# nktoan/h-edit

Hardware: AMD Instinct MI355X
Metric: edited images/sec (512^2, 50 steps, K Langevin) (higher is better)
Workload: dtype bf16

## Files before the change

h-edit_amd/csrc/c_api.hip:

```cpp
#include "../../include/hedit.h"
#include <exception>
#include <map>
#include <mutex>
#include <new>
#include <set>
#include <utility>

#include "common.h"
#include "kernels.h"

static thread_local std::string g_last_error;
void hedit_set_error(const std::string& msg) { g_last_error = msg; }

int hedit_abi_catch() noexcept {
  try {
    try {
      throw;
    } catch (const std::bad_alloc&) {
      g_last_error = "out of host memory inside libhedit_hip";
    } catch (const std::exception& e) {
      g_last_error = std::string("C++ exception inside libhedit_hip: ") + e.what();
    } catch (...) {
      g_last_error = "unknown C++ exception inside libhedit_hip";
    }
// ... 335 lines not shown
                       int B, int N, int heads, int d, const hedit_p2p_plan* plan, float* store, void* stream) try {
  ARG_CHECK(q && k && vt && out && plan, "cross_attn args");
  CrossAttnParams p{};
  p.q = reinterpret_cast<const bf16_t*>(q); p.ldq = ldq;
  p.k = reinterpret_cast<const bf16_t*>(k); p.ldk = ldk;
  p.vt = reinterpret_cast<const bf16_t*>(vt); p.ldvt = (long)ldvt;
  p.out = reinterpret_cast<bf16_t*>(out); p.ldo = ldo;
  p.B = B; p.N = N; p.heads = heads; p.d = d;
  p.n_pairs = plan->n_pairs; p.pair_src = plan->pair_src; p.pair_tar = plan->pair_tar;
  p.mixT = reinterpret_cast<const bf16_t*>(plan->mixT); p.bvec = plan->bvec;
  p.singles = plan->singles; p.n_single = plan->n_single;
  p.store = store;
  return cross_attn_launch(p, S(stream));
} catch (...) { return hedit_abi_catch(); }

int hedit_k_attn_probs(const void* q, int ldq, const void* k, int ldk, float* probs, int B, int N, int M, int kstride,
                       int heads, int d, void* stream) try {
  ARG_CHECK(q && k && probs, "attn_probs args");
  AttnProbsParams p{};
  p.q = reinterpret_cast<const bf16_t*>(q); p.ldq = ldq;
  p.k = reinterpret_cast<const bf16_t*>(k); p.ldk = ldk;
  p.probs = probs; p.B = B; p.N = N; p.M = M; p.kstride = kstride; p.heads = heads; p.d = d;
  return attn_probs_launch(p, S(stream));
} catch (...) { return hedit_abi_catch(); }

int hedit_k_attn_apply(const float* probs, const void* vt, int64_t ldvt, void* out, int ldo, int B, int N, int M,
                       int kstride, int heads, int d, void* stream) try {
  ARG_CHECK(probs && vt && out, "attn_apply args");
  AttnProbsParams p{};
  p.probs = const_cast<float*>(probs);
  p.vt = reinterpret_cast<const bf16_t*>(vt); p.ldvt = (long)ldvt;
  p.out = reinterpret_cast<bf16_t*>(out); p.ldo = ldo;
  p.B = B; p.N = N; p.M = M; p.kstride = kstride; p.heads = heads; p.d = d;
  return attn_apply_launch(p, S(stream));
} catch (...) { return hedit_abi_catch(); }

int hedit_k_pack_conv3x3(const float* w, void* out, int O, int I, void* stream) try {
  ARG_CHECK(w && out, "pack args");
  return pack_conv3x3_launch(w, reinterpret_cast<bf16_t*>(out), O, I, S(stream));
} catch (...) { return hedit_abi_catch(); }

int hedit_k_f32_to_bf16(const float* x, void* y, int64_t n, void* stream) try {
  ARG_CHECK(x && y, "cast args");
  return f32_to_bf16_launch(x, reinterpret_cast<bf16_t*>(y), (long)n, S(stream));
} catch (...) { return hedit_abi_catch(); }

int hedit_k_groupnorm_stats(const void* x, void* y, const float* gamma, const float* beta, int B, int HW, int C, int G,
                            float eps, int silu, void* ws, float* stats, void* stream) try {
  ARG_CHECK(x && y && gamma && beta && ws && stats, "groupnorm_stats args");
  return groupnorm_launch(reinterpret_cast<const bf16_t*>(x), reinterpret_cast<bf16_t*>(y), gamma, beta, B, HW, C, G,
                          eps, silu, reinterpret_cast<float*>(ws), S(stream), stats);
} catch (...) { return hedit_abi_catch(); }

size_t hedit_k_groupnorm_bwd_ws_bytes(int B, int HW, int C) { return groupnorm_bwd_ws_bytes(B, HW, C); }

int hedit_k_groupnorm_bwd(const void* x, const void* dy, const void* add, void* dx, const float* gamma, const float* beta,
                          const float* stats, int B, int HW, int C, int G, int silu, void* ws, void* stream) try {
  ARG_CHECK(x && dy && dx && gamma && beta && stats && ws, "groupnorm_bwd args");
  return groupnorm_bwd_launch(reinterpret_cast<const bf16_t*>(x), reinterpret_cast<const bf16_t*>(dy),
                              reinterpret_cast<const bf16_t*>(add), reinterpret_cast<bf16_t*>(dx), gamma, beta, stats, B, HW, C,
                              G, silu, reinterpret_cast<float*>(ws), S(stream));
} catch (...) { return hedit_abi_catch(); }

int hedit_k_softmax_rows(const float* s, void* p, int64_t rows, int N, float scale, void* stream) try {
  ARG_CHECK(s && p, "softmax_rows args");
  return softmax_rows_launch(s, reinterpret_cast<bf16_t*>(p), (long)rows, N, scale, S(stream));
} catch (...) { return hedit_abi_catch(); }

int hedit_k_softmax_blockdiag(const float* s, void* p, int64_t rows, int T, int ld, float scale, void* stream) try {
  ARG_CHECK(s && p, "softmax_blockdiag args");
  return softmax_blockdiag_launch(s, reinterpret_cast<bf16_t*>(p), (long)rows, T, ld, scale, S(stream));
} catch (...) { return hedit_abi_catch(); }

int hedit_k_softmax_bwd(const void* p, const float* dp, void* ds, int64_t rows, int N, float scale, void* stream) try {
  ARG_CHECK(p && dp && ds, "softmax_bwd args");
  return softmax_bwd_launch(reinterpret_cast<const bf16_t*>(p), dp, reinterpret_cast<bf16_t*>(ds), (long)rows, N, scale, S(stream));
} catch (...) { return hedit_abi_catch(); }

int hedit_k_transpose(const void* src, void* dst, int R, int C, void* stream) try {
  ARG_CHECK(src && dst, "transpose args");
  return transpose_bf16_launch(reinterpret_cast<const bf16_t*>(src), reinterpret_cast<bf16_t*>(dst), R, C, S(stream));
} catch (...) { return hedit_abi_catch(); }

int hedit_k_sum2x2(const void* du, void* dx, int B, int H, int W, int C, void* stream) try {
  ARG_CHECK(du && dx, "sum2x2 args");
  return sum2x2_launch(reinterpret_cast<const bf16_t*>(du), reinterpret_cast<bf16_t*>(dx), B, H, W, C, S(stream));
} catch (...) { return hedit_abi_catch(); }

int hedit_k_pack_conv3x3_dgrad(const float* w, void* out, int O, int I, void* stream) try {
  ARG_CHECK(w && out, "pack args");
  return pack_conv3x3_dgrad_launch(w, reinterpret_cast<bf16_t*>(out), O, I, S(stream));
} catch (...) { return hedit_abi_catch(); }

int hedit_k_pack_conv3x3_s2_dgrad(const float* w, void* out, int O, int I, void* stream) try {
  ARG_CHECK(w && out, "pack args");
  return pack_conv3x3_s2_dgrad_launch(w, reinterpret_cast<bf16_t*>(out), O, I, S(stream));
} catch (...) { return hedit_abi_catch(); }

int hedit_k_conv3x3_s2_dgrad(const void* dy, const void* w_packed, void* dx, int B, int Hin, int Win, int O, int I, void* stream) try {
  ARG_CHECK(dy && w_packed && dx, "conv3x3_s2_dgrad args");
  return conv3x3_s2_dgrad_launch(reinterpret_cast<const bf16_t*>(dy), reinterpret_cast<const bf16_t*>(w_packed),
                                 reinterpret_cast<bf16_t*>(dx), B, Hin, Win, O, I, S(stream));
} catch (...) { return hedit_abi_catch(); }

int hedit_k_slice_add(const void* src, int ld, int off, int c, void* dst, int64_t rows, int accumulate, void* stream) try {
  ARG_CHECK(src && dst && rows >= 0, "slice_add args");
// ... 78 lines not shown
```

h-edit_amd/csrc/kernels.h:

```cpp
#pragma once
#include "common.h"

struct GemmParams {
  const bf16_t* A;
  const bf16_t* W;
  int M, N, K;
  int lda;
  int mode;
  int Hin, Win, Cin, Hout, Wout;
  const float* bias;
  const bf16_t* residual;
  int ldr;
  bf16_t* C;
  int ldc;
  float* partial;
  int splits, kt_per_split;
  int n_fastest;
  const bf16_t* zeros;
  unsigned a_bytes, w_bytes;
  int geglu;
  int asym;
  float* raw_f32;
  int chunk_kt;
  const float *ln_gamma, *ln_beta;
// ... 11 lines not shown
int gemm_pick_splits(int M, int N, int K, int force);
int gemm_canonical_chunk(int M_nom, int N_nom, int K);
int gemm_plan_splits(int M, int N, int K, int chunk_kt);
size_t gemm_partial_bytes(int M, int N, int splits);
int gemm_launch(GemmParams p, int splits, float* partial_ws, hipStream_t st);
bool pgemm_supported(const GemmParams& p, int splits, int bn);
int pgemm_launch(const GemmParams& p, int bn, hipStream_t st);
bool pconv_supported(const GemmParams& p, int splits, int bn);
int pconv_launch(const GemmParams& p, int bn, hipStream_t st);

struct FfnParams {
  const bf16_t* x; long ldx;
  const float* gamma; const float* beta; float eps;
  const bf16_t* stream;
  const float* bias1p;
  const float* bias2;
  bf16_t* out; long ldo;
  int M, C;
  const bf16_t* a; long lda;
  const bf16_t* r2; long ldr2;
  const float* bias_pre; const float* bias_post;
};
struct LinChainParams {
  const bf16_t* a; long lda;
  const bf16_t* r1; long ldr1;
  const float* bias_pre;
  const float* gamma; const float* beta; float eps;
  const bf16_t* stream;
  bf16_t* out_mid; long ldmid;
  bf16_t* out; long ldo;
  int M, C;
  const float* gn_ss; int rows_per_image;
  bf16_t* out_q; long ldq; bf16_t* out_k; long ldk;
};
int lin_chain_launch(const LinChainParams& c, hipStream_t st);
int lin_chain_launch_sched(const LinChainParams& c, int sched, hipStream_t st);
size_t lin_chain_stream_bytes(int layers);
int lin_chain_pack_launch(const float* w, int layer, float scale, int layers, bf16_t* stream, hipStream_t st);
int ffn_fused_channels();
size_t ffn_stream_bytes(int pre, int post);
size_t ffn_bias_bytes();
int ffn_pack_launch(const float* w, int which, int pre, int post, bf16_t* stream, hipStream_t st);
int ffn_pack_bias_launch(const float* b1, float* out, hipStream_t st);
int ffn_fused_launch(const FfnParams& f, hipStream_t st);

#define HEDIT_MAXW 77
#define HEDIT_WPAD 96
#define HEDIT_CTXP 80

size_t groupnorm_ws_bytes(int B, int HW, int C);
int groupnorm_launch(const bf16_t* x, bf16_t* y, const float* gamma, const float* beta, int B,
                     int HW, int C, int G, float eps, int silu, float* ws, hipStream_t st,
                     float* stats = nullptr);
bool groupnorm_from_parts_supported(int HW, int C, int G);
size_t groupnorm_from_parts_ws_bytes(int B);
int groupnorm_from_parts_launch(const bf16_t* x, bf16_t* y, const float* gamma, const float* beta, int B, int HW, int C, int G,
                                float eps, int silu, const float* part_a, int ca, const float* part_b, int cb, float* ws,
                                hipStream_t st);
int groupnorm_affine_launch(const bf16_t* x, const float* gamma, const float* beta, int B, int HW, int C, int G, float eps,
                            float* ws, hipStream_t st, const float** ss_out);
int layernorm_launch(const bf16_t* x, bf16_t* y, const float* gamma, const float* beta, long rows,
                     int C, float eps, hipStream_t st);
bool splitk_reduce_ln_supported(int C);
int splitk_reduce_ln_launch(const float* partial, int splits, const float* bias, const bf16_t* residual, int ldr, bf16_t* out,
                            bf16_t* y, const float* gamma, const float* beta, long rows, int C, float eps, hipStream_t st);
int geglu_launch(const bf16_t* x, bf16_t* y, long rows, int inner, hipStream_t st);
#define HEDIT_ROWMAP_MAX 512
struct RowMap { uint16_t src[HEDIT_ROWMAP_MAX]; };
int concat_launch(const bf16_t* a, int ca, const bf16_t* b, int cb, bf16_t* y, long rows, hipStream_t st,
                  const RowMap* b_map = nullptr, int rows_per_image = 0);
int gather_rows_launch(const void* const* src, void* const* dst, int n, int B, long row_bytes, const RowMap& map, hipStream_t st);
int f32_to_bf16_launch(const float* x, bf16_t* y, long n, hipStream_t st);
int ctx_pad_launch(const float* x, bf16_t* y, int B, int dim, hipStream_t st);
int gemv_launch(const bf16_t* W, const float* x, const float* b0, const float* b1, float* out,
                int N, int K, int silu, hipStream_t st);
int copy_rows_launch(bf16_t* x, const int* src, int B, long row_elems, hipStream_t st);
int timestep_embed_launch(float t, float* out, int dim, hipStream_t st);
int timestep_embed_ddpm_launch(float t, float* out, int dim, hipStream_t st);
int conv_in_launch(const float* x, const float* w, const float* bias, bf16_t* y, int B, int Cin,
                   int H, int W, int Cout, hipStream_t st);
int conv_out_launch(const bf16_t* x, const bf16_t* w, const float* bias, float* y, int B, int H,
                    int W, int C, int Cout, hipStream_t st);
int rows_to_nchw_launch(const float* src, const float* bias, float* dst, int B, long HW, int ld, int Cout, hipStream_t st);
int softmax_rows_launch(const float* s, bf16_t* p, long rows, int N, float scale, hipStream_t st);
int softmax_blockdiag_launch(const float* s, bf16_t* p, long rows, int T, int ld, float scale, hipStream_t st);
int mix1x1_nchw_launch(const float* x, const float* w, const float* bias, float* y, int B, int Cin, int Cout, long HW,
                       float pre_scale, hipStream_t st);
int quant_mean_launch(const bf16_t* h, const float* w, const float* bias, float* y, int B, long HW, int Cm, int Cout, hipStream_t st);
int pack_linear_launch(const float* w, bf16_t* out, long n, float scale, hipStream_t st);
int pack_conv3x3_launch(const float* w_oihw, bf16_t* out, int O, int I, hipStream_t st);
int pack_geglu_rows_launch(const float* w, bf16_t* out_bf16, float* out_f32, int rows, int K, hipStream_t st);

size_t groupnorm_bwd_ws_bytes(int B, int HW, int C);
int groupnorm_bwd_launch(const bf16_t* x, const bf16_t* dy, const bf16_t* add, bf16_t* dx, const float* gamma,
                         const float* beta, const float* stats, int B, int HW, int C, int G, int silu, float* ws,
                         hipStream_t st, bool any_width = false);
int softmax_bwd_launch(const bf16_t* p, const float* dp, bf16_t* ds, long rows, int N, float scale, hipStream_t st);
int transpose_bf16_launch(const bf16_t* src, bf16_t* dst, int R, int C, hipStream_t st);
int sum2x2_launch(const bf16_t* du, bf16_t* dx, int B, int H, int W, int C, hipStream_t st);
int pack_conv3x3_dgrad_launch(const float* w_oihw, bf16_t* out, int O, int I, hipStream_t st);
int pack_linear_t_launch(const float* w, bf16_t* out, int O, int I, hipStream_t st, float scale = 1.f);
int flip_oihw_launch(const float* w, float* out, int O, int I, int k, hipStream_t st);
int layernorm_bwd_launch(const bf16_t* x, const bf16_t* dy, const bf16_t* add, bf16_t* dx, const float* gamma, long rows, int C,
                         float eps, hipStream_t st);
int geglu_bwd_launch(const bf16_t* x, const bf16_t* dy, bf16_t* dx, long rows, int inner, hipStream_t st);

// ... 135 lines not shown
```

h-edit_amd/csrc/norm.hip:

```cpp
#include <stdlib.h>
#include "common.h"
#include "kernels.h"

namespace {


constexpr int GN_MAXV = 2;

__global__ __launch_bounds__(256) void gn_partial_kernel(const bf16_t* __restrict__ x, float* __restrict__ part,
                                                         int HW, int C, int G, int nslab) {
  extern __shared__ float lds[];
  const int CV = C / 8;
  const int slab = blockIdx.x, b = blockIdx.y;
  const int pix_per = (HW + nslab - 1) / nslab;
  const int p0 = slab * pix_per;
  int p1 = p0 + pix_per;
  if (p1 > HW) p1 = HW;
  const int R = CV <= 256 ? 256 / CV : 1;
  const int r = CV <= 256 ? threadIdx.x / CV : 0;
  const int cv0 = CV <= 256 ? threadIdx.x % CV : threadIdx.x;
  const bool active = r < R;
  float s[GN_MAXV][8], q[GN_MAXV][8];
#pragma unroll
  for (int v = 0; v < GN_MAXV; ++v)
// ... 550 lines not shown
#pragma unroll
      for (int j = 0; j < 8; ++j) acc[co] += f[j] * ww[j];
    }
  }
  for (int co = 0; co < Cout; ++co) {
    float v = wave_sum(acc[co]);
    if (lane == 0) y[(((long)b * Cout + co) * H + oy) * Wd + ox] = v + bias[co];
  }
}

__global__ __launch_bounds__(256) void gn_small_kernel(const bf16_t* __restrict__ x, bf16_t* __restrict__ y,
                                                       const float* __restrict__ gamma, const float* __restrict__ beta,
                                                       int HW, int C, int G, float eps, int silu, float* __restrict__ stats) {
  extern __shared__ uint32_t gs_pairs[];
  __shared__ float red[8];
  const int g = blockIdx.x, b = blockIdx.y, tid = threadIdx.x;
  const int cpg = C / G, ppp = cpg / 2;
  const int npair = HW * ppp;
  const uint32_t* xin = reinterpret_cast<const uint32_t*>(x + (long)b * HW * C + g * cpg);
  float s = 0.f, q = 0.f;
  for (int i = tid; i < npair; i += 256) {
    const int pix = i / ppp, j = i - pix * ppp;
    const uint32_t u = xin[(long)pix * (C / 2) + j];
    gs_pairs[i] = u;
    const float a = st_lo(u), c = st_hi(u);
    s += a; s += c;
    q += a * a; q += c * c;
  }
  s = wave_sum(s);
  q = wave_sum(q);
  if ((tid & 63) == 0) { red[(tid >> 6) * 2] = s; red[(tid >> 6) * 2 + 1] = q; }
  __syncthreads();
  s = ((red[0] + red[2]) + red[4]) + red[6];
  q = ((red[1] + red[3]) + red[5]) + red[7];
  const float n = (float)HW * (float)cpg;
  const float m = s / n;
  float var = q / n - m * m;
  var = var < 0.f ? 0.f : var;
  const float rstd = rsqrtf(var + eps);
  if (stats && tid == 0) *reinterpret_cast<float2*>(stats + ((long)b * G + g) * 2) = make_float2(m, rstd);
  uint32_t* yout = reinterpret_cast<uint32_t*>(y + (long)b * HW * C + g * cpg);
  for (int i = tid; i < npair; i += 256) {
    const int pix = i / ppp, j = i - pix * ppp;
    const uint32_t u = gs_pairs[i];
    const int c0 = g * cpg + 2 * j;
    const float sc0 = rstd * gamma[c0], sc1 = rstd * gamma[c0 + 1];
    float a = st_lo(u) * sc0 + (beta[c0] - m * sc0);
    float c = st_hi(u) * sc1 + (beta[c0 + 1] - m * sc1);
    if (silu) { a = silu_f(a); c = silu_f(c); }
    yout[(long)pix * (C / 2) + j] = pack_bf16x2(a, c);
  }
}

__global__ __launch_bounds__(256) void gn_fold_kernel(const float* __restrict__ pa, int npa, const float* __restrict__ pb, int npb,
                                                      float* __restrict__ out, int units, int ppg) {
  __shared__ float red[8];
  const int g = blockIdx.x, b = blockIdx.y, tid = threadIdx.x;
  const int total = units * ppg;
  float s = 0.f, q = 0.f;
  for (int e = tid; e < total; e += 256) {
    const int u = e / ppg, j = e - u * ppg;
    const int pr = g * ppg + j;
    const long row = (long)b * units + u;
    const float2 v = pr < npa ? *reinterpret_cast<const float2*>(pa + (row * npa + pr) * 2)
                              : *reinterpret_cast<const float2*>(pb + (row * npb + (pr - npa)) * 2);
    s += v.x;
    q += v.y;
  }
  s = wave_sum(s);
  q = wave_sum(q);
  if ((tid & 63) == 0) { red[(tid >> 6) * 2] = s; red[(tid >> 6) * 2 + 1] = q; }
  __syncthreads();
  if (tid == 0) {
    s = ((red[0] + red[2]) + red[4]) + red[6];
    q = ((red[1] + red[3]) + red[5]) + red[7];
    *reinterpret_cast<float2*>(out + ((long)b * gridDim.x + g) * 2) = make_float2(s, q);
  }
}

int gn_nslab(int B, int HW, int C) {
  (void)B;
  const int CV = C / 8;
  const int R = CV <= 256 ? 256 / CV : 1;
  int n = HW / (R * 8);
  int cap = HW / 256;
  cap = cap < 32 ? 32 : (cap > 64 ? 64 : cap);
  if (HW >= 512 * 512) cap = 128;
  if (n > cap) n = cap;
  if (n < 1) n = 1;
  return n;
}

}

size_t groupnorm_ws_bytes(int B, int HW, int C) {
  const int nslab = gn_nslab(B, HW, C);
  return ((size_t)B * nslab * 64 * 2 + (size_t)B * C * 2) * sizeof(float);
}

int groupnorm_launch(const bf16_t* x, bf16_t* y, const float* gamma, const float* beta, int B, int HW,
                     int C, int G, float eps, int silu, float* ws, hipStream_t st, float* stats) {
  ARG_CHECK(C % 8 == 0 && C % G == 0 && G <= 64, "groupnorm: C % 8, C % G, G <= 64");
  ARG_CHECK(C / 8 <= 256 * GN_MAXV, "groupnorm: C too large");
  if (HW < 1024 && (C / G) % 2 == 0 && (size_t)HW * (C / G) * 2 <= 60 * 1024) {
    hipLaunchKernelGGL(gn_small_kernel, dim3(G, B), dim3(256), (size_t)HW * (C / G) * 2, st, x, y, gamma, beta, HW, C, G, eps, silu, stats);
    LAUNCH_CHECK();
    return HEDIT_OK;
  }
  const int nslab = gn_nslab(B, HW, C);
  float* part = ws;
  float* ss = ws + (size_t)B * nslab * 64 * 2;
  const int CV = C / 8;
  const int R = CV <= 256 ? 256 / CV : 1;
  const size_t lds = (size_t)R * C * 2 * sizeof(float);
  ARG_CHECK(lds <= 64 * 1024, "groupnorm: LDS");
  hipLaunchKernelGGL(gn_partial_kernel, dim3(nslab, B), dim3(256), lds, st, x, part, HW, C, G, nslab);
  LAUNCH_CHECK();
  const long total_v = (long)B * HW * CV;
  const bool rows_form = CV <= 256 && HW >= 1024;
  if (!rows_form || stats) {
    hipLaunchKernelGGL(gn_finalize_kernel, dim3(B), dim3(256), 0, st, part, gamma, beta, ss, HW, C, G, nslab, eps, stats);
    LAUNCH_CHECK();
  }
  if (rows_form) {
    int ns = (int)(4096 / (B > 0 ? B : 1)) + 1;
    const int max_ns = HW / (R * 8) > 0 ? HW / (R * 8) : 1;
    if (ns > max_ns) ns = max_ns;
    {
      int pix = HW / ns / (4 * R) * (4 * R);
      if (pix < 4 * R) pix = 4 * R;
      ns = (HW + pix - 1) / pix;
    }
    hipLaunchKernelGGL(gn_apply_rows_kernel, dim3(ns, B), dim3(256), 0, st, x, y, part, gamma, beta, HW, C, G, nslab, eps, silu, ns);
    LAUNCH_CHECK();
    return HEDIT_OK;
  }
  hipLaunchKernelGGL(gn_apply_kernel, dim3(ew_grid(total_v)), dim3(256), 0, st, x, y, ss, total_v, HW, C, silu);
  LAUNCH_CHECK();
  return HEDIT_OK;
}

bool groupnorm_from_parts_supported(int HW, int C, int G) {
  return HW >= 1024 && HW % 128 == 0 && C % 8 == 0 && C / 8 <= 256 && C % G == 0 && (C / G) % 2 == 0 && G <= 64;
}
size_t groupnorm_from_parts_ws_bytes(int B) { return (size_t)B * 64 * 2 * sizeof(float); }

int groupnorm_from_parts_launch(const bf16_t* x, bf16_t* y, const float* gamma, const float* beta, int B, int HW, int C, int G,
                                float eps, int silu, const float* part_a, int ca, const float* part_b, int cb, float* ws,
                                hipStream_t st) {
  ARG_CHECK(groupnorm_from_parts_supported(HW, C, G), "groupnorm_from_parts: shape");
  ARG_CHECK(part_a && ca > 0 && ca % 2 == 0 && cb >= 0 && cb % 2 == 0 && ca + cb == C && (cb == 0) == (part_b == nullptr),
            "groupnorm_from_parts: the pair statistics must cover the C channels");
  hipLaunchKernelGGL(gn_fold_kernel, dim3(G, B), dim3(256), 0, st, part_a, ca / 2, part_b, cb / 2, ws, HW / 128, C / G / 2);
  LAUNCH_CHECK();
  const int CV = C / 8, R = 256 / CV;
  int ns = (int)(4096 / (B > 0 ? B : 1)) + 1;
  const int max_ns = HW / (R * 8) > 0 ? HW / (R * 8) : 1;
// ... 342 lines not shown
```

h-edit_amd/hedit/_lib.py:

```python
import ctypes as C
import os

_HERE = os.path.dirname(os.path.abspath(__file__))
STORAGE = os.environ.get("HEDIT_STORAGE", "bf16").lower()
if STORAGE not in ("bf16", "f16"):
    raise ValueError(f"HEDIT_STORAGE must be bf16 or f16, not {STORAGE!r}")
LIB_PATH = os.path.join(_HERE, "libhedit_hip_f16.so" if STORAGE == "f16" else "libhedit_hip.so")
HEDIT_MAX_LEVELS = 8


class UnetCfg(C.Structure):
    _fields_ = [("in_channels", C.c_int), ("out_channels", C.c_int), ("sample_size", C.c_int),
                ("n_levels", C.c_int),
                ("block_out_channels", C.c_int * HEDIT_MAX_LEVELS),
                ("down_has_attn", C.c_int * HEDIT_MAX_LEVELS),
                ("up_has_attn", C.c_int * HEDIT_MAX_LEVELS),
                ("layers_per_block", C.c_int), ("cross_attention_dim", C.c_int),
                ("heads", C.c_int), ("norm_num_groups", C.c_int)]


class VaeCfg(C.Structure):
    _fields_ = [("in_channels", C.c_int), ("latent_channels", C.c_int), ("n_levels", C.c_int),
                ("block_out_channels", C.c_int * 4), ("layers_per_block", C.c_int),
                ("norm_num_groups", C.c_int)]
# ... 226 lines not shown
                                 C.c_void_p]),
    "hedit_k_gemm_ws_bytes": (C.c_size_t, [C.c_int, C.c_int, C.c_int, C.c_int]),
    "hedit_k_gemm_canonical_chunk": (C.c_int, [C.c_int, C.c_int, C.c_int]),
    "hedit_k_gemm_plan_splits": (C.c_int, [C.c_int, C.c_int, C.c_int, C.c_int]),
    "hedit_k_gemm": (C.c_int, [C.c_void_p, C.c_void_p, C.c_void_p, C.c_void_p, C.c_void_p] + [C.c_int] * 13 +
                     [C.c_void_p, C.c_void_p]),
    "hedit_k_conv_gn": (C.c_int, [C.c_void_p, C.c_void_p, C.c_void_p, C.c_void_p, C.c_void_p] + [C.c_int] * 12 +
                        [C.c_void_p, C.c_void_p, C.c_void_p]),
    "hedit_k_groupnorm_from_parts": (C.c_int, [C.c_void_p, C.c_void_p, C.c_void_p, C.c_void_p, C.c_int, C.c_int, C.c_int, C.c_int,
                                               C.c_float, C.c_int, C.c_void_p, C.c_int, C.c_void_p, C.c_int, C.c_void_p, C.c_void_p]),
    "hedit_k_pack_geglu": (C.c_int, [C.c_void_p, C.c_void_p, C.c_void_p, C.c_void_p, C.c_int, C.c_int, C.c_void_p]),
    "hedit_k_gemm_geglu": (C.c_int, [C.c_void_p, C.c_void_p, C.c_void_p, C.c_void_p, C.c_int, C.c_int, C.c_int,
                                     C.c_int, C.c_int, C.c_void_p]),
    "hedit_test_set_flags": (C.c_int, [C.c_int]),
    "hedit_storage_is_f16": (C.c_int, []),
    "hedit_k_lin_chain_stream_bytes": (C.c_size_t, [C.c_int]),
    "hedit_k_lin_chain_pack": (C.c_int, [C.c_void_p, C.c_void_p, C.c_void_p, C.c_void_p, C.c_float, C.c_void_p, C.c_void_p]),
    "hedit_k_lin_chain": (C.c_int, [C.c_void_p, C.c_int64, C.c_void_p, C.c_int64, C.c_void_p, C.c_int, C.c_void_p, C.c_void_p, C.c_void_p,
                                    C.c_float, C.c_void_p, C.c_void_p, C.c_int64, C.c_void_p, C.c_int64, C.c_void_p, C.c_int64,
                                    C.c_void_p, C.c_int64, C.c_int, C.c_int, C.c_void_p]),
    "hedit_k_lin_chain_sched": (C.c_int, [C.c_void_p, C.c_int64, C.c_void_p, C.c_int64, C.c_void_p, C.c_int, C.c_void_p, C.c_void_p, C.c_void_p,
                                          C.c_float, C.c_void_p, C.c_void_p, C.c_int64, C.c_void_p, C.c_int64, C.c_void_p, C.c_int64,
                                          C.c_void_p, C.c_int64, C.c_int, C.c_int, C.c_int, C.c_void_p]),
    "hedit_k_groupnorm_affine": (C.c_int, [C.c_void_p, C.c_void_p, C.c_void_p, C.c_int, C.c_int, C.c_int, C.c_int, C.c_float, C.c_void_p,
                                           C.c_void_p, C.c_void_p]),
    "hedit_k_ffn_channels": (C.c_int, []),
    "hedit_k_ffn_stream_bytes": (C.c_size_t, [C.c_int]),
    "hedit_k_ffn_bias_bytes": (C.c_size_t, []),
    "hedit_k_ffn_pack": (C.c_int, [C.c_void_p, C.c_void_p, C.c_void_p, C.c_void_p, C.c_void_p, C.c_void_p, C.c_void_p, C.c_void_p]),
    "hedit_k_ffn_chain": (C.c_int, [C.c_void_p, C.c_int64, C.c_void_p, C.c_int64, C.c_void_p, C.c_int64, C.c_void_p, C.c_void_p, C.c_void_p,
                                    C.c_float, C.c_void_p, C.c_void_p, C.c_void_p, C.c_void_p, C.c_void_p, C.c_int64, C.c_int, C.c_int,
                                    C.c_void_p]),
    "hedit_k_ffn_fused": (C.c_int, [C.c_void_p, C.c_int64, C.c_void_p, C.c_void_p, C.c_float, C.c_void_p, C.c_void_p,
                                    C.c_void_p, C.c_void_p, C.c_int64, C.c_int, C.c_int, C.c_void_p]),
    "hedit_k_groupnorm_ws_bytes": (C.c_size_t, [C.c_int, C.c_int, C.c_int]),
    "hedit_k_groupnorm": (C.c_int, [C.c_void_p, C.c_void_p, C.c_void_p, C.c_void_p, C.c_int, C.c_int, C.c_int,
                                    C.c_int, C.c_float, C.c_int, C.c_void_p, C.c_void_p]),
    "hedit_k_layernorm": (C.c_int, [C.c_void_p, C.c_void_p, C.c_void_p, C.c_void_p, C.c_int64, C.c_int,
                                    C.c_float, C.c_void_p]),
    "hedit_k_geglu": (C.c_int, [C.c_void_p, C.c_void_p, C.c_int64, C.c_int, C.c_void_p]),
    "hedit_k_self_attn": (C.c_int, [C.c_void_p, C.c_int, C.c_void_p, C.c_int, C.c_void_p, C.c_int64, C.c_void_p,
                                    C.c_int, C.c_int, C.c_int, C.c_int, C.c_int, C.c_void_p, C.c_void_p, C.c_void_p]),
    "hedit_k_cross_attn": (C.c_int, [C.c_void_p, C.c_int, C.c_void_p, C.c_int, C.c_void_p, C.c_int64, C.c_void_p,
                                     C.c_int, C.c_int, C.c_int, C.c_int, C.c_int, C.POINTER(P2PPlan), C.c_void_p,
                                     C.c_void_p]),
    "hedit_k_attn_probs": (C.c_int, [C.c_void_p, C.c_int, C.c_void_p, C.c_int, C.c_void_p, C.c_int, C.c_int, C.c_int, C.c_int,
                                     C.c_int, C.c_int, C.c_void_p]),
    "hedit_k_attn_apply": (C.c_int, [C.c_void_p, C.c_void_p, C.c_int64, C.c_void_p, C.c_int, C.c_int, C.c_int, C.c_int, C.c_int,
                                     C.c_int, C.c_int, C.c_void_p]),
    "hedit_k_pack_conv3x3": (C.c_int, [C.c_void_p, C.c_void_p, C.c_int, C.c_int, C.c_void_p]),
    "hedit_k_f32_to_bf16": (C.c_int, [C.c_void_p, C.c_void_p, C.c_int64, C.c_void_p]),
    "hedit_k_groupnorm_stats": (C.c_int, [C.c_void_p, C.c_void_p, C.c_void_p, C.c_void_p, C.c_int, C.c_int, C.c_int,
                                          C.c_int, C.c_float, C.c_int, C.c_void_p, C.c_void_p, C.c_void_p]),
    "hedit_k_groupnorm_bwd_ws_bytes": (C.c_size_t, [C.c_int, C.c_int, C.c_int]),
    "hedit_k_groupnorm_bwd": (C.c_int, [C.c_void_p] * 7 + [C.c_int] * 5 + [C.c_void_p, C.c_void_p]),
    "hedit_k_softmax_rows": (C.c_int, [C.c_void_p, C.c_void_p, C.c_int64, C.c_int, C.c_float, C.c_void_p]),
    "hedit_k_softmax_blockdiag": (C.c_int, [C.c_void_p, C.c_void_p, C.c_int64, C.c_int, C.c_int, C.c_float, C.c_void_p]),
    "hedit_k_softmax_bwd": (C.c_int, [C.c_void_p, C.c_void_p, C.c_void_p, C.c_int64, C.c_int, C.c_float, C.c_void_p]),
    "hedit_k_transpose": (C.c_int, [C.c_void_p, C.c_void_p, C.c_int, C.c_int, C.c_void_p]),
    "hedit_k_sum2x2": (C.c_int, [C.c_void_p, C.c_void_p, C.c_int, C.c_int, C.c_int, C.c_int, C.c_void_p]),
    "hedit_k_pack_conv3x3_dgrad": (C.c_int, [C.c_void_p, C.c_void_p, C.c_int, C.c_int, C.c_void_p]),
    "hedit_k_pack_conv3x3_s2_dgrad": (C.c_int, [C.c_void_p, C.c_void_p, C.c_int, C.c_int, C.c_void_p]),
    "hedit_k_conv3x3_s2_dgrad": (C.c_int, [C.c_void_p, C.c_void_p, C.c_void_p, C.c_int, C.c_int, C.c_int, C.c_int, C.c_int,
                                           C.c_void_p]),
    "hedit_k_slice_add": (C.c_int, [C.c_void_p, C.c_int, C.c_int, C.c_int, C.c_void_p, C.c_int64, C.c_int, C.c_void_p]),
    "hedit_k_pack_linear_t": (C.c_int, [C.c_void_p, C.c_void_p, C.c_int, C.c_int, C.c_void_p]),
    "hedit_k_flip_oihw": (C.c_int, [C.c_void_p, C.c_void_p, C.c_int, C.c_int, C.c_int, C.c_void_p]),
    "hedit_k_attn_bwd_ws_bytes": (C.c_size_t, [C.c_int, C.c_int, C.c_int]),
    "hedit_k_attn_bwd": (C.c_int, [C.c_void_p, C.c_int] * 6 + [C.c_void_p, C.c_void_p] + [C.c_int] * 4 + [C.c_void_p, C.c_void_p]),
    "hedit_k_cross_attn_bwd_q": (C.c_int, [C.c_void_p, C.c_int] * 6 + [C.c_int] * 4 + [C.c_void_p]),
    "hedit_k_layernorm_bwd": (C.c_int, [C.c_void_p] * 5 + [C.c_int64, C.c_int, C.c_float, C.c_void_p]),
    "hedit_k_groupnorm_bwd_any": (C.c_int, [C.c_void_p] * 7 + [C.c_int] * 5 + [C.c_void_p, C.c_void_p]),
    "hedit_k_geglu_bwd": (C.c_int, [C.c_void_p, C.c_void_p, C.c_void_p, C.c_int64, C.c_int, C.c_void_p]),
    "hedit_k_conv3x3_s2_dgrad_pad1": (C.c_int, [C.c_void_p, C.c_void_p, C.c_void_p, C.c_int, C.c_int, C.c_int, C.c_int, C.c_int,
                                                C.c_void_p]),
}

EXPORTS = tuple(_SIGS.keys())


class HipLibraryMissing(RuntimeError):
    pass


_lib = None


def lib():
    global _lib
    if _lib is None:
        if not os.path.exists(LIB_PATH):
            raise HipLibraryMissing(
                f"{LIB_PATH} not found: build it with `python h-edit_amd/build.py{' --f16' if STORAGE == 'f16' else ''}` "
                "(hipcc --offload-arch=gfx950); hedit has no CPU/eager fallback")
        l = C.CDLL(LIB_PATH)
        for name, (res, args) in _SIGS.items():
            fn = getattr(l, name)
            fn.restype = res
            fn.argtypes = args
        if bool(l.hedit_storage_is_f16()) != (STORAGE == "f16"):
            raise HipLibraryMissing(f"{LIB_PATH} was not built for HEDIT_STORAGE={STORAGE}")
        _lib = l
    return _lib


def storage_dtype():
# ... 21 lines not shown
```

include/hedit.h:

```cpp
#ifndef HEDIT_H
#define HEDIT_H
#include <stddef.h>
#include <stdint.h>

#ifdef __cplusplus
extern "C" {
#endif

#define HEDIT_MAX_LEVELS 8

typedef struct hedit_unet hedit_unet;

typedef struct {
  int in_channels, out_channels, sample_size;
  int n_levels;
  int block_out_channels[HEDIT_MAX_LEVELS];
  int down_has_attn[HEDIT_MAX_LEVELS];
  int up_has_attn[HEDIT_MAX_LEVELS];
  int layers_per_block;
  int cross_attention_dim;
  int heads;
  int norm_num_groups;
} hedit_unet_cfg;

// ... 125 lines not shown
                    void* stream);
int hedit_k_groupnorm_from_parts(const void* x, void* y, const float* gamma, const float* beta, int B, int HW, int C, int G,
                                 float eps, int silu, const float* part_a, int ca, const float* part_b, int cb, void* ws,
                                 void* stream);
int hedit_k_pack_geglu(const float* w, const float* bias, void* w_packed_bf16, float* bias_packed,
                       int inner, int K, void* stream);
int hedit_k_gemm_geglu(const void* A, const void* w_packed, const float* bias_packed, void* C, int M,
                       int inner, int K, int lda, int ldc, void* stream);
int hedit_k_ffn_channels(void);
size_t hedit_k_ffn_stream_bytes(int with_outer_layers);
size_t hedit_k_ffn_bias_bytes(void);
int hedit_k_ffn_pack(const float* w1, const float* b1, const float* w2, const float* w_pre, const float* w_post, void* stream_out,
                     float* bias1_out, void* stream);
int hedit_k_ffn_fused(const void* x, int64_t ldx, const float* gamma, const float* beta, float eps, const void* w_stream,
                      const float* bias1_packed, const float* bias2, void* out, int64_t ldo, int M, int C, void* stream);
int hedit_k_ffn_chain(const void* a, int64_t lda, const void* t1, int64_t ldt1, const void* x, int64_t ldx, const float* bias_pre,
                      const float* gamma, const float* beta, float eps, const void* w_stream, const float* bias1_packed,
                      const float* bias2, const float* bias_post, void* out, int64_t ldo, int M, int C, void* stream);
size_t hedit_k_lin_chain_stream_bytes(int n_out);
int hedit_k_lin_chain_pack(const float* w_pre, const float* w0, const float* w1, const float* w2, float scale0, void* stream_out,
                           void* stream);
int hedit_k_lin_chain(const void* a, int64_t lda, const void* r1, int64_t ldr1, const float* gn_ss, int rows_per_image,
                      const float* bias_pre, const float* gamma, const float* beta, float eps, const void* w_stream, void* out_mid,
                      int64_t ldmid, void* out_q, int64_t ldq, void* out_k, int64_t ldk, void* out, int64_t ldo, int M, int C,
                      void* stream);
int hedit_k_lin_chain_sched(const void* a, int64_t lda, const void* r1, int64_t ldr1, const float* gn_ss, int rows_per_image,
                            const float* bias_pre, const float* gamma, const float* beta, float eps, const void* w_stream, void* out_mid,
                            int64_t ldmid, void* out_q, int64_t ldq, void* out_k, int64_t ldk, void* out, int64_t ldo, int M, int C,
                            int sched, void* stream);
int hedit_storage_is_f16(void);
int hedit_test_set_flags(int flags);
size_t hedit_k_groupnorm_ws_bytes(int B, int HW, int C);
int hedit_k_groupnorm_affine(const void* x, const float* gamma, const float* beta, int B, int HW, int C, int G, float eps, void* ws,
                             float* ss_out, void* stream);
int hedit_k_groupnorm(const void* x, void* y, const float* gamma, const float* beta, int B, int HW,
                      int C, int G, float eps, int silu, void* ws, void* stream);
int hedit_k_layernorm(const void* x, void* y, const float* gamma, const float* beta, int64_t rows,
                      int C, float eps, void* stream);
int hedit_k_geglu(const void* x, void* y, int64_t rows, int inner, void* stream);
int hedit_k_self_attn(const void* q, int ldq, const void* k, int ldk, const void* vt, int64_t ldvt,
                      void* out, int ldo, int B, int N, int heads, int d, const int32_t* qk_src, const int32_t* kv_src,
                      void* stream);
int hedit_k_cross_attn(const void* q, int ldq, const void* k, int ldk, const void* vt, int64_t ldvt,
                       void* out, int ldo, int B, int N, int heads, int d,
                       const hedit_p2p_plan* plan, float* store, void* stream);
int hedit_k_attn_probs(const void* q, int ldq, const void* k, int ldk, float* probs, int B, int N, int M, int kstride,
                       int heads, int d, void* stream);
int hedit_k_attn_apply(const float* probs, const void* vt, int64_t ldvt, void* out, int ldo, int B, int N, int M,
                       int kstride, int heads, int d, void* stream);
int hedit_k_pack_conv3x3(const float* w_oihw, void* out, int O, int I, void* stream);
int hedit_k_f32_to_bf16(const float* x, void* y, int64_t n, void* stream);
int hedit_k_groupnorm_stats(const void* x, void* y, const float* gamma, const float* beta, int B, int HW, int C, int G,
                            float eps, int silu, void* ws, float* stats, void* stream);
size_t hedit_k_groupnorm_bwd_ws_bytes(int B, int HW, int C);
int hedit_k_groupnorm_bwd(const void* x, const void* dy, const void* add, void* dx, const float* gamma, const float* beta,
                          const float* stats, int B, int HW, int C, int G, int silu, void* ws, void* stream);
int hedit_k_softmax_rows(const float* s, void* p, int64_t rows, int N, float scale, void* stream);
int hedit_k_softmax_blockdiag(const float* s, void* p, int64_t rows, int T, int ld, float scale, void* stream);
int hedit_k_softmax_bwd(const void* p, const float* dp, void* ds, int64_t rows, int N, float scale, void* stream);
int hedit_k_transpose(const void* src, void* dst, int R, int C, void* stream);
int hedit_k_sum2x2(const void* du, void* dx, int B, int H, int W, int C, void* stream);
int hedit_k_pack_conv3x3_dgrad(const float* w_oihw, void* out, int O, int I, void* stream);
int hedit_k_pack_linear_t(const float* w, void* out, int O, int I, void* stream);
int hedit_k_flip_oihw(const float* w_oihw, float* out, int O, int I, int k, void* stream);
int hedit_k_pack_conv3x3_s2_dgrad(const float* w_oihw, void* out, int O, int I, void* stream);
int hedit_k_conv3x3_s2_dgrad(const void* dy, const void* w_packed, void* dx, int B, int Hin, int Win, int O, int I, void* stream);
int hedit_k_slice_add(const void* src, int ld, int off, int c, void* dst, int64_t rows, int accumulate, void* stream);
size_t hedit_k_attn_bwd_ws_bytes(int B, int N, int heads);
int hedit_k_attn_bwd(const void* q, int ldq, const void* k, int ldk, const void* v, int ldv, const void* o, int ldo,
                     const void* dout, int lddo, void* dq, int lddq, void* dk, void* dv, int B, int N, int heads, int d,
                     void* ws, void* stream);
int hedit_k_cross_attn_bwd_q(const void* q, int ldq, const void* k, int ldk, const void* v, int ldv, const void* o, int ldo,
                             const void* dout, int lddo, void* dq, int lddq, int B, int N, int heads, int d, void* stream);
int hedit_k_layernorm_bwd(const void* x, const void* dy, const void* add, void* dx, const float* gamma, int64_t rows, int C,
                          float eps, void* stream);
int hedit_k_groupnorm_bwd_any(const void* x, const void* dy, const void* add, void* dx, const float* gamma, const float* beta,
                              const float* stats, int B, int HW, int C, int G, int silu, void* ws, void* stream);
int hedit_k_geglu_bwd(const void* x, const void* dy, void* dx, int64_t rows, int inner, void* stream);
int hedit_k_conv3x3_s2_dgrad_pad1(const void* dy, const void* w_packed, void* dx, int B, int Hin, int Win, int O, int I,
                                  void* stream);

typedef struct hedit_ddpm hedit_ddpm;
typedef struct {
  int in_channels, out_ch, ch, n_levels;
  int ch_mult[8];
  int attn_level[8];
  int num_res_blocks, image_size;
} hedit_ddpm_cfg;
int hedit_ddpm_create(const hedit_ddpm_cfg* cfg, hedit_ddpm** out);
void hedit_ddpm_destroy(hedit_ddpm* h);
int hedit_ddpm_num_params(const hedit_ddpm* h);
const char* hedit_ddpm_param_name(const hedit_ddpm* h, int i);
int hedit_ddpm_param_shape(const hedit_ddpm* h, int i, int* ndim, int* dims4);
int hedit_ddpm_load(hedit_ddpm* h, const char* name, const float* dev_w, size_t numel, void* stream);
int hedit_ddpm_missing(const hedit_ddpm* h);
size_t hedit_ddpm_workspace_bytes(hedit_ddpm* h, int B);
int hedit_ddpm_forward(hedit_ddpm* h, const float* x, float t, int B, float* eps, void* workspace,
                       size_t workspace_bytes, void* stream);
int hedit_ddpm_create_grad(const hedit_ddpm_cfg* cfg, hedit_ddpm** out);
size_t hedit_ddpm_grad_workspace_bytes(hedit_ddpm* h, int B);
int hedit_ddpm_forward_keep(hedit_ddpm* h, const float* x, float t, int B, float* eps, void* workspace,
                            size_t workspace_bytes, void* stream);
int hedit_ddpm_backward(hedit_ddpm* h, const float* d_eps, float* d_x, void* workspace, void* stream);
void hedit_ddpm_release(hedit_ddpm* h);
int hedit_ddpm_vjp(hedit_ddpm* h, const float* x, float t, const float* d_eps, int B, float* d_x, float* eps, void* workspace,
                   size_t workspace_bytes, void* stream);
// ... 134 lines not shown
```

Before: 2.633.

## Add multi-group LDS-resident GroupNorm kernel for small spatial sizes

```diff
diff --git a/h-edit_amd/csrc/c_api.hip b/h-edit_amd/csrc/c_api.hip
--- a/h-edit_amd/csrc/c_api.hip
+++ b/h-edit_amd/csrc/c_api.hip
@@ -411,6 +411,14 @@
                           eps, silu, reinterpret_cast<float*>(ws), S(stream), stats);
 } catch (...) { return hedit_abi_catch(); }
 
+int hedit_k_groupnorm_small_ref(const void* x, void* y, const float* gamma, const float* beta, int B, int HW, int C, int G,
+                                float eps, int silu, void* ws, float* stats, void* stream) try {
+  ARG_CHECK(x && y && gamma && beta, "groupnorm_small_ref args");
+  (void)ws;
+  return groupnorm_small_ref_launch(reinterpret_cast<const bf16_t*>(x), reinterpret_cast<bf16_t*>(y), gamma, beta, B, HW, C, G,
+                                    eps, silu, S(stream), stats);
+} catch (...) { return hedit_abi_catch(); }
+
 size_t hedit_k_groupnorm_bwd_ws_bytes(int B, int HW, int C) { return groupnorm_bwd_ws_bytes(B, HW, C); }
 
 int hedit_k_groupnorm_bwd(const void* x, const void* dy, const void* add, void* dx, const float* gamma, const float* beta,
diff --git a/h-edit_amd/csrc/kernels.h b/h-edit_amd/csrc/kernels.h
--- a/h-edit_amd/csrc/kernels.h
+++ b/h-edit_amd/csrc/kernels.h
@@ -87,6 +87,8 @@
 int groupnorm_launch(const bf16_t* x, bf16_t* y, const float* gamma, const float* beta, int B,
                      int HW, int C, int G, float eps, int silu, float* ws, hipStream_t st,
                      float* stats = nullptr);
+int groupnorm_small_ref_launch(const bf16_t* x, bf16_t* y, const float* gamma, const float* beta, int B, int HW, int C, int G,
+                               float eps, int silu, hipStream_t st, float* stats);
 bool groupnorm_from_parts_supported(int HW, int C, int G);
 size_t groupnorm_from_parts_ws_bytes(int B);
 int groupnorm_from_parts_launch(const bf16_t* x, bf16_t* y, const float* gamma, const float* beta, int B, int HW, int C, int G,
diff --git a/h-edit_amd/csrc/norm.hip b/h-edit_amd/csrc/norm.hip
--- a/h-edit_amd/csrc/norm.hip
+++ b/h-edit_amd/csrc/norm.hip
@@ -626,6 +626,128 @@
   }
 }
 
+constexpr int GN_RES_INFLIGHT = 8;
+constexpr int GN_RES_MIN = 16 * 1024;
+constexpr int GN_RES_LDS = 40 * 1024;
+constexpr int GN_RES_LDS_MAX = 80 * 1024;
+constexpr int GN_RES_MAXG = 32;
+
+__global__ __launch_bounds__(256) void gn_resident_kernel(const bf16_t* __restrict__ x, bf16_t* __restrict__ y,
+                                                          const float* __restrict__ gamma, const float* __restrict__ beta,
+                                                          int HW, int C, int G, int GPB, float eps, int silu,
+                                                          float* __restrict__ stats) {
+  extern __shared__ uint4 gr_slab[];
+  int b, gb;
+  {
+    const int nblk = G / GPB, id = blockIdx.x, full = (int)gridDim.x / nblk / 8 * 8;
+    if (id < full * nblk) {
+      const int chunk = id / (8 * nblk), within = id - chunk * (8 * nblk);
+      b = chunk * 8 + (within & 7);
+      gb = within >> 3;
+    } else {
+      const int rest = id - full * nblk;
+      b = full + rest / nblk;
+      gb = rest - rest / nblk * nblk;
+    }
+  }
+  const int tid = threadIdx.x, lane = tid & 63, wave = tid >> 6;
+  const int g0 = gb * GPB;
+  const int cpg = C / G, ppp = cpg / 2;
+  const int VPP = GPB * cpg / 8;
+  const int R = 256 / VPP;
+  const int r = tid / VPP, cv = tid - r * VPP;
+  const bool active = r < R;
+  const long base = (long)b * HW * C + (long)g0 * cpg + cv * 8;
+  if (active) {
+    const bf16_t* xg = x + base;
+    for (int p0 = r; p0 < HW; p0 += GN_RES_INFLIGHT * R) {
+      uint4 u[GN_RES_INFLIGHT];
+#pragma unroll
+      for (int k = 0; k < GN_RES_INFLIGHT; ++k) {
+        int p = p0 + k * R;
+        p = p < HW ? p : HW - 1;
+        u[k] = *reinterpret_cast<const uint4*>(xg + (long)p * C);
+      }
+#pragma unroll
+      for (int k = 0; k < GN_RES_INFLIGHT; ++k) {
+        const int p = p0 + k * R;
+        if (p < HW) gr_slab[p * VPP + cv] = u[k];
+      }
+    }
+  }
+  __syncthreads();
+  uint4 first = make_uint4(0u, 0u, 0u, 0u);
+  if (active && r < HW) first = gr_slab[tid];
+  const uint32_t* words = reinterpret_cast<const uint32_t*>(gr_slab);
+  const int wpp = VPP * 4;
+  const int npair = HW * ppp;
+  const int dpix = 256 / ppp, dj = 256 - dpix * ppp;
+  const int pix0 = tid / ppp, j0 = tid - pix0 * ppp;
+  float ks = 0.f, kq = 0.f;
+  for (int gl = 0; gl < GPB; ++gl) {
+    const uint32_t* wg = words + gl * ppp;
+    float s = 0.f, q = 0.f;
+    int pix = pix0, j = j0;
+#pragma unroll 4
+    for (int i = tid; i < npair; i += 256) {
+      const uint32_t u = wg[pix * wpp + j];
+      const float a = st_lo(u), c = st_hi(u);
+      s += a; s += c;
+      q += a * a; q += c * c;
+      pix += dpix;
+      j += dj;
+      if (j >= ppp) { j -= ppp; ++pix; }
+    }
+    s = wave_sum(s);
+    q = wave_sum(q);
+    if (lane == gl) { ks = s; kq = q; }
+  }
+  __syncthreads();
+  float* red = reinterpret_cast<float*>(gr_slab);
+  if (lane < GPB) { red[lane * 8 + wave * 2] = ks; red[lane * 8 + wave * 2 + 1] = kq; }
+  __syncthreads();
+  const float n = (float)HW * (float)cpg;
+  auto group_stats = [&](int gl, float& m, float& rstd) __attribute__((always_inline)) {
+    const float* rg = red + gl * 8;
+    const float s = ((rg[0] + rg[2]) + rg[4]) + rg[6];
+    const float q = ((rg[1] + rg[3]) + rg[5]) + rg[7];
+    m = s / n;
+    float var = q / n - m * m;
+    var = var < 0.f ? 0.f : var;
+    rstd = rsqrtf(var + eps);
+  };
+  if (stats && tid < GPB) {
+    float m, rstd;
+    group_stats(tid, m, rstd);
+    *reinterpret_cast<float2*>(stats + ((long)b * G + g0 + tid) * 2) = make_float2(m, rstd);
+  }
+  if (!active) return;
+  float sc[8], sh[8];
+#pragma unroll
+  for (int j = 0; j < 8; ++j) {
+    const int cl = cv * 8 + j, c = g0 * cpg + cl;
+    float m, rstd;
+    group_stats(cl / cpg, m, rstd);
+    sc[j] = rstd * gamma[c];
+    sh[j] = beta[c] - m * sc[j];
+  }
+  bf16_t* yg = y + base;
+  auto one = [&](const uint4& u, int p) __attribute__((always_inline)) {
+    float f[8];
+    unpack8(u, f);
+#pragma unroll
+    for (int j = 0; j < 8; ++j) f[j] = f[j] * sc[j] + sh[j];
+    if (silu) {
+#pragma unroll
+      for (int j = 0; j < 8; ++j) f[j] = silu_f(f[j]);
+    }
+    *reinterpret_cast<uint4*>(yg + (long)p * C) = pack8(f);
+  };
+  if (r < HW) one(first, r);
+#pragma unroll 4
+  for (int p = r + R; p < HW; p += R) one(gr_slab[p * VPP + cv], p);
+}
+
 __global__ __launch_bounds__(256) void gn_fold_kernel(const float* __restrict__ pa, int npa, const float* __restrict__ pb, int npb,
                                                       float* __restrict__ out, int units, int ppg) {
   __shared__ float red[8];
@@ -665,6 +787,31 @@
   return n;
 }
 
+bool gn_small_ok(int HW, int C, int G) { return HW < 1024 && (C / G) % 2 == 0 && (size_t)HW * (C / G) * 2 <= 60 * 1024; }
+
+int gn_res_gpb(int HW, int C, int G) {
+  if (!gn_small_ok(HW, C, G)) return 0;
+  const int gbytes = C / G * 2;
+  if ((long)HW * gbytes < GN_RES_MIN) return 0;
+  int best = 0, least = 0;
+  for (int gpb = 1; gpb <= G && gpb <= GN_RES_MAXG; ++gpb) {
+    const long slab = (long)HW * gpb * gbytes;
+    if (G % gpb || (gpb * gbytes) % 16 || gpb * gbytes / 16 > 256 || slab > GN_RES_LDS_MAX) continue;
+    if (slab <= GN_RES_LDS) best = gpb;
+    if (!least) least = gpb;
+  }
+  return best ? best : least;
+}
+
+}
+
+int groupnorm_small_ref_launch(const bf16_t* x, bf16_t* y, const float* gamma, const float* beta, int B, int HW, int C, int G,
+                               float eps, int silu, hipStream_t st, float* stats) {
+  ARG_CHECK(C % 8 == 0 && C % G == 0 && G <= 64, "groupnorm: C % 8, C % G, G <= 64");
+  ARG_CHECK(gn_small_ok(HW, C, G), "groupnorm_small_ref: HW < 1024, C / G even, one group of one image within 60 KB");
+  hipLaunchKernelGGL(gn_small_kernel, dim3(G, B), dim3(256), (size_t)HW * (C / G) * 2, st, x, y, gamma, beta, HW, C, G, eps, silu, stats);
+  LAUNCH_CHECK();
+  return HEDIT_OK;
 }
 
 size_t groupnorm_ws_bytes(int B, int HW, int C) {
@@ -676,7 +823,15 @@
                      int C, int G, float eps, int silu, float* ws, hipStream_t st, float* stats) {
   ARG_CHECK(C % 8 == 0 && C % G == 0 && G <= 64, "groupnorm: C % 8, C % G, G <= 64");
   ARG_CHECK(C / 8 <= 256 * GN_MAXV, "groupnorm: C too large");
-  if (HW < 1024 && (C / G) % 2 == 0 && (size_t)HW * (C / G) * 2 <= 60 * 1024) {
+  if (const int gpb = gn_res_gpb(HW, C, G)) {
+    const int slab = HW * gpb * (C / G) * 2, red = gpb * 8 * (int)sizeof(float);
+    if (int rc = hedit_dyn_lds(reinterpret_cast<const void*>(&gn_resident_kernel), GN_RES_LDS_MAX)) return rc;
+    hipLaunchKernelGGL(gn_resident_kernel, dim3(G / gpb * B), dim3(256), (size_t)(slab > red ? slab : red), st, x, y,
+                       gamma, beta, HW, C, G, gpb, eps, silu, stats);
+    LAUNCH_CHECK();
+    return HEDIT_OK;
+  }
+  if (gn_small_ok(HW, C, G)) {
     hipLaunchKernelGGL(gn_small_kernel, dim3(G, B), dim3(256), (size_t)HW * (C / G) * 2, st, x, y, gamma, beta, HW, C, G, eps, silu, stats);
     LAUNCH_CHECK();
     return HEDIT_OK;
diff --git a/h-edit_amd/hedit/_lib.py b/h-edit_amd/hedit/_lib.py
--- a/h-edit_amd/hedit/_lib.py
+++ b/h-edit_amd/hedit/_lib.py
@@ -302,6 +302,8 @@
     "hedit_k_f32_to_bf16": (C.c_int, [C.c_void_p, C.c_void_p, C.c_int64, C.c_void_p]),
     "hedit_k_groupnorm_stats": (C.c_int, [C.c_void_p, C.c_void_p, C.c_void_p, C.c_void_p, C.c_int, C.c_int, C.c_int,
                                           C.c_int, C.c_float, C.c_int, C.c_void_p, C.c_void_p, C.c_void_p]),
+    "hedit_k_groupnorm_small_ref": (C.c_int, [C.c_void_p, C.c_void_p, C.c_void_p, C.c_void_p, C.c_int, C.c_int, C.c_int,
+                                              C.c_int, C.c_float, C.c_int, C.c_void_p, C.c_void_p, C.c_void_p]),
     "hedit_k_groupnorm_bwd_ws_bytes": (C.c_size_t, [C.c_int, C.c_int, C.c_int]),
     "hedit_k_groupnorm_bwd": (C.c_int, [C.c_void_p] * 7 + [C.c_int] * 5 + [C.c_void_p, C.c_void_p]),
     "hedit_k_softmax_rows": (C.c_int, [C.c_void_p, C.c_void_p, C.c_int64, C.c_int, C.c_float, C.c_void_p]),
diff --git a/include/hedit.h b/include/hedit.h
--- a/include/hedit.h
+++ b/include/hedit.h
@@ -201,6 +201,8 @@
 int hedit_k_f32_to_bf16(const float* x, void* y, int64_t n, void* stream);
 int hedit_k_groupnorm_stats(const void* x, void* y, const float* gamma, const float* beta, int B, int HW, int C, int G,
                             float eps, int silu, void* ws, float* stats, void* stream);
+int hedit_k_groupnorm_small_ref(const void* x, void* y, const float* gamma, const float* beta, int B, int HW, int C, int G,
+                                float eps, int silu, void* ws, float* stats, void* stream);
 size_t hedit_k_groupnorm_bwd_ws_bytes(int B, int HW, int C);
 int hedit_k_groupnorm_bwd(const void* x, const void* dy, const void* add, void* dx, const float* gamma, const float* beta,
                           const float* stats, int B, int HW, int C, int G, int silu, void* ws, void* stream);
```

Result: no change. 2.645 (median of 6 runs) (+0.5%).
